# Julia-Tempering/Pigeons.jl

Hardware: AMD Instinct MI355X
Metric: replica-steps/sec (explore+swap), toy_mvn d=1024, n_chains=1024; round-trip rate (higher is better)
Workload: dtype f64

## Files before the change

pigeons.jl_amd/csrc/pte_slice8.hpp:

```cpp
#pragma once
#include "pte_slice7.hpp"

namespace pte {

#ifndef PTE_S8_BD
#define PTE_S8_BD 3
#endif
#ifndef PTE_S8_BS
#define PTE_S8_BS 9
#endif
constexpr int S8_BD = PTE_S8_BD;

#ifndef PTE_S8_WAVES
#define PTE_S8_WAVES 4
#endif
template <int NLU, int S8_BS, int WINDOW, int DBL_MODE>
__device__ __forceinline__ void slice8_body(EngineDev e, SliceParams sp, const int64_t cl) {
    using namespace s7;
    constexpr int WIN = WINDOW, REFILL_AT = WINDOW - PTE_S7_MARGIN;
    constexpr bool FAST = (DBL_MODE == 2);
    static_assert(CAP_ITERS >= S8_BS, "lane 0 must be able to run past the speculative budget");
#ifndef PTE_S8_BLK
#define PTE_S8_BLK 256
#endif
    constexpr int BLK = PTE_S8_BLK, CPB = BLK / 64;
    __shared__ struct {
        double u[WIN];
        double e[WIN];
        double x[BLK];
        double we[256];
        unsigned long long ke[256];
    } sm;
    double (&s_u)[WIN] = sm.u; double (&s_e)[WIN] = sm.e; double (&s_x)[BLK] = sm.x; double (&s_we)[256] = sm.we; unsigned long long (&s_ke)[256] = sm.ke;
    const int lane = lane_id();
#ifdef PTE_PROFILE_WAVES
    const uint64_t wave_t0 = __builtin_amdgcn_s_memrealtime();
#endif
    for (int i = lane; i < 256; i += 64) { s_we[i] = ZIG_WE[i]; s_ke[i] = ZIG_KE[i]; }
    __syncthreads();
    if (cl >= e.K) return;
    const int64_t c = e.c0 + cl;
    const int slot = e.slot_of_chain[cl];
    if (is_ref_chain(e, c)) {
        iid_refresh_recorded<NLU>(e, cl, c, slot, e.sd[c], lane);
        return;
    }
    const double lp_before = lp_before_explore(e, c, slot);
    const int64_t d = e.d;
    double *xrow = e.x + (int64_t)slot * e.ld;
    const int B = (int)((d + 63) >> 6);
    const double nhp = e.nhp[c];
    const double inv_nhp = 1.0 / nhp;
    const double inv_abs_nhp = -inv_nhp * (1.0 + 1e-6);
    const double w = sp.w;
    const double w11 = 1.1 * sp.w;
    const int cap_iters = min(sp.max_iter, CAP_ITERS);
    const int kcap = min(sp.p, 20);
    const bool shr_more = S8_BS < cap_iters;
    constexpr bool HAND_SHRINK = (S8_BS == PTE_S8_BS && S8_BS >= 6 && S8_BS <= 10);
    constexpr bool N_IS_KN = (DBL_MODE == 2) && HAND_SHRINK;

    const int hg = s7_level(lane);
    const int hrel = s7_pick(LO, hg, 0) + lane - s7_pick(BASE, hg, 0);

    const int succ_lo = s7_pick(LO, hg + 1, 0), succ_wd = s7_pick(WD, hg + 1, 0), succ_base = s7_pick(BASE, hg + 1, 0);
    const int succ_off = hrel - succ_lo;
    const int word_c = 0x10000 - succ_off;
    const int word_c9 = (1 << 20) - succ_off * 512;
    const uint64_t seed_in = e.rng[2 * slot];

    double BS = 0.0;
    for (int b = 0; b < B; ++b) {
        int64_t i = 64 * (int64_t)b + lane;
        double v = (i < d) ? xrow[i] : 0.0;
        double s = wave_sum_dpp(v * v);
        if (lane == b) BS = s;
    }
    double S = upper_tree_root<NLU>(BS);
    if (nhp * S == -INFINITY) { if (lane == 0) set_error(e, ERR_SLICE_SUPPORT, (int)c, -1); return; }

    uint64_t wseed = e.rng[2 * slot];
    const uint64_t gamma = e.rng[2 * slot + 1];
    int p = 0;
    uint64_t gamma_inv = gamma;
    for (int k = 0; k < 5; ++k) gamma_inv *= 2ull - gamma * gamma_inv;
    double wsum = 0.0;
    typedef unsigned mask2_t __attribute__((ext_vector_type(2)));
    typedef unsigned slow_mask_t __attribute__((ext_vector_type(WIN / 32)));
    slow_mask_t slow_w;
    auto fill_window = [&]() __attribute__((always_inline)) {
        __syncthreads();
        double acc = 0.0;
#pragma unroll
        for (int k = 0; k < WIN / 64; ++k) {
            const int i = 64 * k + lane;
            const uint64_t r = mix64(wseed + (uint64_t)(i + 1) * gamma);
            const uint64_t ri = r & MASK52;
            const int idx = (int)(ri & 0xFF);
            const bool fast = ri < s_ke[idx];
            const double ev = (double)ri * s_we[idx];
            s_u[i] = u52_to_unit(r);
            s_e[i] = fast ? ev : __longlong_as_double(0x7ff8000000000000LL);
            acc += fast ? ev : 0.0;
            const uint64_t sb = ballot64(!fast);
            slow_w[2 * k] = (unsigned)sb; slow_w[2 * k + 1] = (unsigned)(sb >> 32);
        }
        wsum = wave_sum_dpp(acc);
        p = 0;
        __syncthreads();
    };
    fill_window();

    int dbl_z0 = 0, dbl_z1 = 0, dbl_one_hi = 0x3ff00000;
    if constexpr (DBL_MODE == 2) asm volatile("" : "+v"(dbl_z0), "+v"(dbl_z1), "+v"(dbl_one_hi));

    long long steps_sum = 0, fb_draws = 0, ex_total = 0;
    int steps_n = 0, acc_sum = 0, acc_n = 0, n_fb = 0;
    int err = 0, err_coord = -1;
#ifdef PTE_PROFILE_SECTIONS
    long long prof[16] = {0, 0, 0, 0, 0, 0, 0, 0, 0, 0, 0, 0, 0, 0, 0, 0};
#endif

    for (int pass = 0; pass < sp.n_passes && !err; ++pass) {
        for (int b = 0; BLK * (int64_t)b < d && !err; ++b) {
            const int64_t base = BLK * (int64_t)b;
            const int nl = (int)min((int64_t)BLK, d - base);
#pragma unroll
            for (int k = 0; k < CPB; ++k) s_x[64 * k + lane] = (64 * k + lane < nl) ? xrow[base + 64 * k + lane] : 0.0;
            __builtin_amdgcn_wave_barrier();
            double Sest = S * (1.0 + 1e-6) + wsum * inv_abs_nhp;
            int l = 0, l_end = nl;
            do {
                PROF_T(t0);
                if (__builtin_expect(p > REFILL_AT, 0)) { wseed += (uint64_t)p * gamma; fill_window(); Sest = Sest * (1.0 + 1e-6) + wsum * inv_abs_nhp; }
                const bool active = (l + hg) < nl;
                const double xold = s_x[(l + hg) & (BLK - 1)];
                int idx0 = p + hrel;
                double E = s_e[idx0];
                double u0 = s_u[idx0 + 1];
                double Vd[S8_BD];
#pragma unroll
                for (int it = 0; it < S8_BD; ++it) Vd[it] = s_u[idx0 + 2 + it];
                int ex0 = 0;
                int cnt_base = 2;
                asm volatile("" : "+v"(cnt_base));
                unsigned slow_b;
                if constexpr (WIN == 512)
                    asm("s_lshr_b32 m0, %[p], 5\n" "s_nop 0\n" "s_movrels_b32 %[o], s84\n" "s_lshr_b32 %[o], %[o], %[p]"
                        : [o] "=&s"(slow_b) : [p] "s"(p), "{s[84:99]}"(slow_w) : "m0", "scc");
                else
                    asm("s_lshr_b32 m0, %[p], 5\n" "s_nop 0\n" "s_movrels_b32 %[o], s84\n" "s_lshr_b32 %[o], %[o], %[p]"
                        : [o] "=&s"(slow_b) : [p] "s"(p), "{s[84:91]}"(slow_w) : "m0", "scc");
                static_assert(WIN == 512 || WIN == 256, "the slow-path mask is sixteen or eight dwords");
                if (__builtin_expect((slow_b & 1u) != 0u, 0)) {
                    SeqRng rs{wseed + (uint64_t)p * gamma, gamma};
                    const double Ex = randexp_seq(rs);
                    const int used = (int)((rs.seed - (wseed + (uint64_t)p * gamma)) * gamma_inv);
                    if (used <= 17) {
                        ex0 = used - 1;
                        if (lane == 0) { E = Ex; idx0 += ex0; cnt_base = 2 + ex0; }
                        Sest += Ex * inv_abs_nhp;
                        ex_total += ex0;
                        u0 = s_u[idx0 + 1];
#pragma unroll
                        for (int it = 0; it < S8_BD; ++it) Vd[it] = s_u[idx0 + 2 + it];
                    }
                }
                const double Enh = E * inv_nhp;
                const double Q = __builtin_fma(xold, xold, -Enh);
                const double Bq = Sest + fabs(Q);
                double dmin = fabs(Enh);
                auto test = [&](double v) __attribute__((always_inline)) -> double {
                    const double d = __builtin_fma(v, v, -Q);
                    dmin = fmin(dmin, fabs(d));
                    return d;
                };
                double LL = xold - w * u0;
                double RR = LL + w;
                double dL = test(LL), dR = test(RR);
                int kd = 0;
                double dmin_lr = 0.0;
                unsigned need_l0 = 0u;
                uint64_t need_m = 0ull;
#if PTE_S8_BD >= 1 && PTE_S8_BD <= 4 && !defined(PTE_S8_DOUBLING_SELECTS)
                if constexpr (DBL_MODE == 2) {
                    double t_, wd_;
                    int sLh_, sRh_;
                    uint64_t sv_, sx_;
                    mask2_t sd_;
#define PTE_S8_CSTEP(V) \
                    "v_cmp_ge_f64 vcc, 0.5, " V "\n" \
                    "v_min_f64 v[102:103], v[114:115], v[116:117]\n" \
                    "v_cmpx_gt_f64_e64 %[sx], 0, v[102:103]\n" \
                    "v_add_f64 v[112:113], v[98:99], -v[96:97]\n" \
                    "v_add_u32 %[kd], 1, %[kd]\n" \
                    "v_cndmask_b32 v119, 0, %[one], vcc\n" \
                    "v_cndmask_b32 v121, %[one], v118, vcc\n" \
                    "v_fma_f64 v[96:97], -v[118:119], v[112:113], v[96:97]\n" \
                    "v_fma_f64 v[98:99], v[120:121], v[112:113], v[98:99]\n" \
                    "v_fma_f64 v[114:115], v[96:97], v[96:97], -v[110:111]\n" \
                    "v_fma_f64 v[116:117], v[98:99], v[98:99], -v[110:111]\n" \
                    "v_min_f64 v[104:105], v[104:105], |v[114:115]|\n" \
                    "v_min_f64 v[104:105], v[104:105], |v[116:117]|\n"
                    asm volatile("s_mov_b64 %[sv], exec\n"
                                 PTE_S8_CSTEP("%[V0]")
#if PTE_S8_BD >= 2
                                 PTE_S8_CSTEP("%[V1]")
#endif
#if PTE_S8_BD >= 3
                                 PTE_S8_CSTEP("%[V2]")
#endif
#if PTE_S8_BD >= 4
                                 PTE_S8_CSTEP("%[V3]")
#endif
                                 "s_mov_b64 exec, %[sv]\n"
                                 "v_min_f64 v[102:103], v[114:115], v[116:117]\n"
                                 "v_cmp_gt_f64_e64 %[sd], 0, v[102:103]\n"
                                 : "+{v[96:97]}"(LL), "+{v[98:99]}"(RR), "+{v[114:115]}"(dL), "+{v[116:117]}"(dR), "+{v[104:105]}"(dmin), [kd] "+v"(kd),
                                   "=&{v[102:103]}"(t_), "=&{v[112:113]}"(wd_), "=&{v119}"(sLh_), "=&{v121}"(sRh_), [sv] "=&s"(sv_), [sx] "=&s"(sx_), [sd] "=&s"(sd_)
                                 : "{v[110:111]}"(Q), "{v118}"(dbl_z0), "{v120}"(dbl_z1), [one] "v"(dbl_one_hi),
                                   [V0] "v"(Vd[0]), [V1] "v"(Vd[S8_BD > 1 ? 1 : 0]), [V2] "v"(Vd[S8_BD > 2 ? 2 : 0]), [V3] "v"(Vd[S8_BD > 3 ? 3 : 0])
                                 : "vcc", "scc");
#undef PTE_S8_CSTEP
                    dmin_lr = t_;
                    need_m = (uint64_t)sd_.x | ((uint64_t)sd_.y << 32); need_l0 = __builtin_amdgcn_readfirstlane(sd_.x);
                } else
                if (DBL_MODE == 1 && sp.p >= S8_BD) {
                    double t_, wd_;
                    uint64_t sv_, sv2_;
#define PTE_S8_DSTEP(V) \
                    "v_min_f64 %[t], %[dL], %[dR]\n" \
                    "v_cmp_gt_f64 vcc, 0, %[t]\n" \
                    "s_and_saveexec_b64 %[sv], vcc\n" \
                    "v_add_u32 %[kd], 1, %[kd]\n" \
                    "v_add_f64 %[wd], %[RR], -%[LL]\n" \
                    "v_cmp_ge_f64 vcc, 0.5, " V "\n" \
                    "s_and_saveexec_b64 %[sv2], vcc\n" \
                    "v_add_f64 %[LL], %[LL], -%[wd]\n" \
                    "v_fma_f64 %[dL], %[LL], %[LL], -%[Q]\n" \
                    "v_min_f64 %[dmin], %[dmin], |%[dL]|\n" \
                    "s_andn2_b64 exec, %[sv2], exec\n" \
                    "v_add_f64 %[RR], %[RR], %[wd]\n" \
                    "v_fma_f64 %[dR], %[RR], %[RR], -%[Q]\n" \
                    "v_min_f64 %[dmin], %[dmin], |%[dR]|\n" \
                    "s_mov_b64 exec, %[sv]\n"
                    asm volatile(PTE_S8_DSTEP("%[V0]")
#if PTE_S8_BD >= 2
                                 PTE_S8_DSTEP("%[V1]")
#endif
#if PTE_S8_BD >= 3
                                 PTE_S8_DSTEP("%[V2]")
#endif
#if PTE_S8_BD >= 4
                                 PTE_S8_DSTEP("%[V3]")
#endif
                                 : [LL] "+v"(LL), [RR] "+v"(RR), [dL] "+v"(dL), [dR] "+v"(dR), [dmin] "+v"(dmin), [kd] "+v"(kd),
                                   [t] "=&v"(t_), [wd] "=&v"(wd_), [sv] "=&s"(sv_), [sv2] "=&s"(sv2_)
                                 : [Q] "v"(Q), [V0] "v"(Vd[0]), [V1] "v"(Vd[S8_BD > 1 ? 1 : 0]), [V2] "v"(Vd[S8_BD > 2 ? 2 : 0]), [V3] "v"(Vd[S8_BD > 3 ? 3 : 0])
                                 : "vcc", "scc");
#undef PTE_S8_DSTEP
                } else
#endif
#pragma unroll
                for (int it = 0; it < S8_BD; ++it) {
                    const bool need = (fmin(dL, dR) < 0.0) && it < sp.p;
                    const double V = Vd[it];
                    kd += need ? 1 : 0;
                    const bool left = V <= 0.5;
                    const double wd = RR - LL;
                    if constexpr (DBL_MODE == 0) {
                        const double sL = (need && left) ? 1.0 : 0.0, sR = (need && !left) ? 1.0 : 0.0;
                        LL = __builtin_fma(-sL, wd, LL);
                        RR = __builtin_fma(sR, wd, RR);
                        dL = __builtin_fma(LL, LL, -Q);
                        dR = __builtin_fma(RR, RR, -Q);
                        dmin = fmin(dmin, fmin(fabs(dL), fabs(dR)));
                    } else {
                        const double cand = left ? (LL - wd) : (RR + wd);
                        const double dc = __builtin_fma(cand, cand, -Q);
                        dmin = need ? fmin(dmin, fabs(dc)) : dmin;
                        const bool nl_ = need && left, nr_ = need && !left;
                        LL = nl_ ? cand : LL;
                        RR = nr_ ? cand : RR;
                        dL = nl_ ? dc : dL;
                        dR = nr_ ? dc : dR;
                    }
                }
#if !(PTE_S8_BD >= 1 && PTE_S8_BD <= 4) || defined(PTE_S8_DOUBLING_SELECTS)
                static_assert(DBL_MODE != 2, "PTE_S8_DBL_MODE == 2 needs the v_cmpx doubling block: 1 <= PTE_S8_BD <= 4 and no PTE_S8_DOUBLING_SELECTS");
#endif
                if constexpr (DBL_MODE != 2) dmin_lr = fmin(dL, dR);
                unsigned more_dbl;
                if constexpr (FAST) more_dbl = need_l0 & 1u;
                else more_dbl = ballot64(lane == 0 && (dmin_lr < 0.0) && kd < kcap) != 0ull ? 1u : 0u;
                if (__builtin_expect(more_dbl != 0u, 0)) {
                    bool need = (lane == 0);
                    while (need) {
                        const double V = s_u[idx0 + 2 + kd];
                        kd += 1;
                        const bool left = V <= 0.5;
                        const double wd = RR - LL;
                        const double cand = left ? (LL - wd) : (RR + wd);
                        const double dc = test(cand);
                        LL = left ? cand : LL;
                        RR = left ? RR : cand;
                        dL = left ? dc : dL;
                        dR = left ? dR : dc;
                        need = (kd < kcap) && (fmin(dL, dR) < 0.0);
                    }
                    asm volatile("" : "+v"(dL), "+v"(dR), "+v"(kd));
                    dmin_lr = fmin(dL, dR);
                    if constexpr (FAST) {
                        dmin_lr = (kd >= sp.p) ? 0.0 : dmin_lr;
                        need_m = ballot64(dmin_lr < 0.0);
                        need_l0 = (unsigned)need_m;
                    }
                }
                const bool dbl_ok = FAST ? !__builtin_amdgcn_inverse_ballot_w64(need_m) : !((kd < sp.p) && (dmin_lr < 0.0));
                double thr2 = 1e-6 * fmax(fabs(LL), fabs(RR));
                if constexpr (DBL_MODE == 2) asm volatile("" : "+v"(thr2));
#ifdef PTE_PROFILE_SECTIONS
                asm volatile("" :: "v"(LL), "v"(RR), "v"(kd), "v"(thr2));
#endif
                PROF_T(t1); PROF_ADD(0, t1 - t0);
                const double *us = &s_u[idx0 + 2 + kd];
                double u[S8_BS];
#pragma unroll
                for (int k = 0; k < S8_BS; ++k) u[k] = us[k];
                double mthr = 2e-12 * Bq;
                int kn0 = cnt_base + kd + succ_off;
                uint64_t pre_ok;
                if constexpr (FAST) pre_ok = ballot64(active) & ~need_m;
                else pre_ok = ballot64(active && dbl_ok);
                double Lbar = LL, Rbar = RR, xf = xold, W = 0.0;
                int n = N_IS_KN ? kn0 : 0;
                if constexpr (FAST) {
                    if constexpr (N_IS_KN) asm volatile("" : "+v"(mthr), "+v"(n), "+s"(pre_ok));
                    else asm volatile("" : "+v"(mthr), "+v"(kn0), "+s"(pre_ok));
                }
                bool fin = false;
                unsigned unf_l0 = 0u;
                uint64_t unf_m = 0ull;
                if constexpr (S8_BS == PTE_S8_BS && S8_BS >= 6 && S8_BS <= 10) {
                    double t_;
                    mask2_t unf_mask;
                    uint64_t exec_save;
#define PTE_S8_STEP(U) \
                    "v_add_f64 v[112:113], v[98:99], -v[96:97]\n" \
                    "v_mul_f64 v[102:103], " U ", v[112:113]\n" \
                    "v_add_f64 v[100:101], v[96:97], v[102:103]\n" \
                    "v_cmp_lt_f64 vcc, v[100:101], v[108:109]\n" \
                    "v_fma_f64 v[102:103], v[100:101], v[100:101], -v[110:111]\n" \
                    "v_add_u32 v106, 1, v106\n" \
                    "v_cndmask_b32 v96, v96, v100, vcc\n" \
                    "v_cndmask_b32 v97, v97, v101, vcc\n" \
                    "v_cndmask_b32 v98, v100, v98, vcc\n" \
                    "v_cndmask_b32 v99, v101, v99, vcc\n" \
                    "v_min_f64 v[104:105], v[104:105], |v[102:103]|\n" \
                    "v_cmpx_ngt_f64 vcc, 0, v[102:103]\n"
                    asm volatile(".p2align 3\n"
                                 "s_mov_b64 %[sv], exec\n"
                                 PTE_S8_STEP("%[u0]") PTE_S8_STEP("%[u1]") PTE_S8_STEP("%[u2]") PTE_S8_STEP("%[u3]")
                                 PTE_S8_STEP("%[u4]") PTE_S8_STEP("%[u5]")
#if PTE_S8_BS >= 7
                                 PTE_S8_STEP("%[u6]")
#endif
#if PTE_S8_BS >= 8
                                 PTE_S8_STEP("%[u7]")
#endif
#if PTE_S8_BS >= 9
                                 PTE_S8_STEP("%[u8]")
#endif
#if PTE_S8_BS >= 10
                                 PTE_S8_STEP("%[u9]")
#endif
                                 "s_mov_b64 %[unf], exec\n"
                                 "s_mov_b64 exec, %[sv]\n"
                                 "s_nop 3\n"
                                 : "+{v[96:97]}"(Lbar), "+{v[98:99]}"(Rbar), "=&{v[100:101]}"(xf), "=&{v[102:103]}"(t_),
                                   "+{v[104:105]}"(dmin), "+{v106}"(n), "=&{v[112:113]}"(W), [unf] "=&s"(unf_mask), [sv] "=&s"(exec_save)
                                 : "{v[108:109]}"(xold), "{v[110:111]}"(Q), [u0] "v"(u[0]), [u1] "v"(u[1]), [u2] "v"(u[2]), [u3] "v"(u[3]),
                                   [u4] "v"(u[4]), [u5] "v"(u[5]), [u6] "v"(u[S8_BS > 6 ? 6 : 0]), [u7] "v"(u[S8_BS > 7 ? 7 : 0]),
                                   [u8] "v"(u[S8_BS > 8 ? 8 : 0]), [u9] "v"(u[S8_BS > 9 ? 9 : 0])
                                 : "vcc");
#undef PTE_S8_STEP
                    unf_m = (uint64_t)unf_mask.x | ((uint64_t)unf_mask.y << 32); unf_l0 = __builtin_amdgcn_readfirstlane(unf_mask.x);
                    fin = !__builtin_amdgcn_inverse_ballot_w64(unf_m);
                } else {
#pragma unroll
                    for (int k = 0; k < S8_BS; ++k) {
                        W = Rbar - Lbar;
                        const double v = Lbar + u[k] * W;
                        const double dv = __builtin_fma(v, v, -Q);
                        dmin = fmin(dmin, fabs(dv));
                        xf = fin ? xf : v;
                        n += fin ? 0 : 1;
                        const bool below = v < xold;
                        Lbar = below ? v : Lbar;
                        Rbar = below ? Rbar : v;
                        fin = fin || (dv < 0.0);
                    }
                    unf_m = ballot64(!fin);
                    unf_l0 = (unsigned)unf_m;
                }
                if (__builtin_expect((unf_l0 & 1u) != 0u, 0)) {
                  if (shr_more) {
                    double dx = 1.0;
                    bool go = (lane == 0);
                    const int n_off = N_IS_KN ? cnt_base + kd + succ_off : 0;
                    while (go) {
                        W = Rbar - Lbar;
                        xf = Lbar + us[n - n_off] * W;
                        n += 1;
                        dx = test(xf);
                        const bool below = xf < xold;
                        Lbar = below ? xf : Lbar;
                        Rbar = below ? Rbar : xf;
                        go = !(dx < 0.0) && n - n_off < cap_iters;
                    }
                    asm volatile("" : "+v"(dx), "+v"(n), "+v"(W));
                    fin = fin || (lane == 0 && dx < 0.0);
                    unf_m = ballot64(!fin);
                  }
                }
                PROF_T(t2); PROF_ADD(1, t2 - t1); PROF_ADD(3, 1);
                int gdone;
#ifdef PTE_PROFILE_SECTIONS
                constexpr bool ASM_TAIL = false;
#else
                constexpr bool ASM_TAIL = FAST && G == 5;
#endif
                if constexpr (ASM_TAIL) {
                    const int kn = N_IS_KN ? n : kn0 + n;
                    const int wsucc = ((unsigned)kn < (unsigned)succ_wd) ? kn + succ_base : 0;
                    const int word_v = (kn << 9) + word_c9 + wsucc;
                    unsigned acc; uint64_t tmask, sA_, sB_; int w_, pk_, s0_, s1_, s2_, s3_, s4_;
                    asm volatile("v_cmp_gt_f64 vcc, %[W], %[thr]\n"
                                 "v_cndmask_b32_e64 %[w], 0, %[wv], %[pre]\n"
                                 "v_cmp_gt_f64_e64 %[sA], %[dm], %[mthr]\n"
                                 "v_cndmask_b32_e64 %[w], %[w], 0, %[unf]\n"
                                 "v_cndmask_b32_e32 %[w], 0, %[w], vcc\n"
                                 "s_nop 0\n"
                                 "v_cndmask_b32_e64 %[w], 0, %[w], %[sA]\n"
                                 "v_cndmask_b32_e64 %[pk], 0, %[w], %[nz]\n"
                                 : [w] "=&v"(w_), [pk] "=&v"(pk_), [sA] "=&s"(sA_)
                                 : [wv] "v"(word_v), [pre] "s"(pre_ok), [unf] "s"(unf_m), [nz] "s"(0xFFFFFFFFFFFFFFFEull),
                                   [W] "v"(W), [thr] "v"(thr2), [dm] "v"(dmin), [mthr] "v"(mthr)
                                 : "vcc");
                    asm volatile("v_cmp_ne_u32_e64 %[sB], 0, %[w]\n"
                                 "s_mov_b64 %[tm], 1\n"
                                 "v_readlane_b32 %[s0], %[w], 0\n"
                                 "s_nop 3\n"
                                 "v_readlane_b32 %[s1], %[pk], %[s0]\n"
                                 "s_bitset1_b64 %[tm], %[s0]\n"
                                 "s_mov_b32 %[acc], %[s0]\n"
                                 "s_nop 1\n"
                                 "v_readlane_b32 %[s2], %[pk], %[s1]\n"
                                 "s_bitset1_b64 %[tm], %[s1]\n"
                                 "s_add_u32 %[acc], %[acc], %[s1]\n"
                                 "s_nop 1\n"
                                 "v_readlane_b32 %[s3], %[pk], %[s2]\n"
                                 "s_bitset1_b64 %[tm], %[s2]\n"
                                 "s_add_u32 %[acc], %[acc], %[s2]\n"
                                 "s_nop 1\n"
                                 "v_readlane_b32 %[s4], %[pk], %[s3]\n"
                                 "s_bitset1_b64 %[tm], %[s3]\n"
                                 "s_add_u32 %[acc], %[acc], %[s3]\n"
                                 "s_and_b64 %[tm], %[tm], %[sB]\n"
                                 "s_add_u32 %[acc], %[acc], %[s4]\n"
                                 : [sB] "=&s"(sB_), [tm] "=&s"(tmask), [acc] "=&s"(acc),
                                   [s0] "=&s"(s0_), [s1] "=&s"(s1_), [s2] "=&s"(s2_), [s3] "=&s"(s3_), [s4] "=&s"(s4_)
                                 : [w] "v"(w_), [pk] "v"(pk_)
                                 : "scc");
                    if (__builtin_amdgcn_inverse_ballot_w64(tmask)) s_x[(l + hg) & (BLK - 1)] = xf;
                    __builtin_amdgcn_wave_barrier();
                    p += (int)((acc >> 9) & 0x1FFu);
                    gdone = (int)((acc >> 20) & 7u);
                    l += gdone;
                } else {
                bool valid = __builtin_amdgcn_inverse_ballot_w64(pre_ok) && fin && (W > thr2);
                if constexpr (!FAST) valid = valid && !(E != E) && n <= cap_iters;
#ifdef PTE_PROFILE_SECTIONS
                asm volatile("" :: "v"(xf), "v"(n), "v"(dmin));
#endif
#ifdef PTE_PROFILE_SECTIONS
                {
                    const bool mg = dmin > 2e-12 * Bq;
                    const int rc = !active ? 7 : (E != E) ? 1 : !dbl_ok ? 2 : !fin ? 3 : !valid ? 4 : !mg ? 5 : 0;
                    const int cnt_ = N_IS_KN ? n - succ_off : cnt_base + kd + n;
                    int o_ = 0, g_ = 0, why = 0;
                    for (g_ = 0; g_ < G; ++g_) {
                        if (l + g_ >= nl) { why = 7; break; }
                        const int k_ = o_ - LO[g_];
                        if ((unsigned)k_ >= (unsigned)WD[g_]) { why = 6; break; }
                        const int ln_ = BASE[g_] + k_;
                        const int r_ = __builtin_amdgcn_readlane(rc, ln_);
                        if (r_) { why = r_; break; }
                        o_ += __builtin_amdgcn_readlane(cnt_, ln_);
                    }
                    PROF_ADD(8 + why, 1);
                }
#endif
                valid = valid && (dmin > mthr);
                const int kn = N_IS_KN ? n : kn0 + n;
                const bool inw = (unsigned)kn < (unsigned)succ_wd;
                const uint64_t vmask = ballot64(valid);
                int word_v = kn + word_c + (inw ? (int)((unsigned)(kn + succ_base) << 24) : 0);
                asm("" : "+v"(word_v));
                const int word = valid ? word_v : 0;
                const int packed = (lane != 0) ? word : 0;
#ifdef PTE_PROFILE_SECTIONS
                asm volatile("" :: "v"(packed));
#endif
                {
                    int pk = __builtin_amdgcn_readlane(word, 0);
                    unsigned acc = 0u;
                    uint64_t tmask = 1ull;
#pragma unroll
                    for (int g = 1; g < G; ++g) {
                        const int cur = (int)((unsigned)pk >> 24);
                        asm volatile("s_bitset1_b64 %0, %2\n\ts_add_u32 %1, %1, %3" : "+s"(tmask), "+s"(acc) : "s"(cur), "s"(pk) : "scc");
                        pk = __builtin_amdgcn_readlane(packed, cur);
                    }
                    acc += (unsigned)pk;
                    tmask &= vmask;
                    if (__builtin_amdgcn_inverse_ballot_w64(tmask)) s_x[(l + hg) & (BLK - 1)] = xf;
                    __builtin_amdgcn_wave_barrier();
                    p += (int)(acc & 0xFFFFu);
                    gdone = (int)((acc >> 16) & 0xFFu);
                    l += gdone;
                }
                }
#ifdef PTE_PROFILE_SECTIONS
                asm volatile("" :: "s"(p), "s"(l));
#endif
                PROF_T(t4); PROF_ADD(5, t4 - t2); PROF_ADD(4, gdone);
                if (__builtin_expect(gdone == 0, 0)) {
                    ex_total -= ex0;
                    SeqRng rs{wseed + (uint64_t)p * gamma, gamma};
                    const int ck = l >> 6, li = l & 63, bc = CPB * b + ck;
#pragma unroll
                    for (int k = 0; k < CPB; ++k) {
                        const double xk = s_x[64 * k + lane];
                        const double sk = wave_sum_dpp(xk * xk);
                        if (lane == CPB * b + k) BS = sk;
                    }
                    const double X = s_x[64 * ck + lane];
                    const double xo = readlane_f64(X, li);
                    const double E = randexp_seq(rs);
                    const double u0 = rs.rand();
                    const double Q = xo * xo - E * inv_nhp;
                    const double mg = 1e-12 * (Sest + fabs(Q));
                    const double Qlo = Q - mg, Qhi = Q + mg;
                    auto inside_exact = [&](double v) __attribute__((always_inline)) -> bool {
                        const double Xv = (lane == li) ? v : X;
                        const double sv = wave_sum_dpp(Xv * Xv), s0 = wave_sum_dpp(X * X);
                        const double Sv = upper_tree_root<NLU>((lane == bc) ? sv : BS);
                        const double S0 = upper_tree_root<NLU>((lane == bc) ? s0 : BS);
                        const double zz = nhp * S0 - E;
                        return zz < nhp * Sv;
                    };
                    auto inside = [&](double v) __attribute__((always_inline)) -> bool {
                        const double q = v * v;
                        const bool in = q < Qlo;
                        const bool out = q > Qhi;
                        if (__builtin_expect(!(in || out), 0)) return inside_exact(v);
                        return in;
                    };
                    double LL = xo - w * u0;
                    double RR = LL + w;
                    bool in_L = inside(LL), in_R = inside(RR);
                    int K = sp.p;
                    while (K > 0 && (in_L || in_R)) {
                        const double V = rs.rand();
                        if (V <= 0.5) { LL = LL - (RR - LL); in_L = inside(LL); }
                        else { RR = RR + (RR - LL); in_R = inside(RR); }
                        K -= 1;
                    }
                    steps_sum += (sp.p - K); steps_n += 1;
                    const bool doubled = (RR - LL) > w11;
                    double Lbar = LL, Rbar = RR;
                    double xn = xo;
                    bool fin = false;
                    for (int n = 1; n <= sp.max_iter; ++n) {
                        const double newpos = Lbar + rs.rand() * (Rbar - Lbar);
                        if (inside(newpos)) {
                            bool ok = true;
                            if (doubled) {
                                double Lhat = LL, Rhat = RR;
                                bool oL = !in_L, oR = !in_R;
                                bool Rstale = false, Lstale = false, D = false;
                                while (Rhat - Lhat > w11) {
                                    const double Mid = (Lhat + Rhat) / 2.0;
                                    if ((xo < Mid && newpos >= Mid) || (xo >= Mid && newpos < Mid)) D = true;
                                    if (newpos < Mid) { Rhat = Mid; Rstale = true; }
                                    else { Lhat = Mid; Lstale = true; }
                                    if (D) {
                                        if (Lstale) { oL = !inside(Lhat); Lstale = false; }
                                        if (Rstale) { oR = !inside(Rhat); Rstale = false; }
                                        if (oL && oR) { ok = false; break; }
                                    }
                                }
                            }
                            acc_n += 1;
                            if (ok) { acc_sum += 1; xn = newpos; steps_sum += n; steps_n += 1; fin = true; break; }
                        }
                        if (newpos < xo) Lbar = newpos; else Rbar = newpos;
                        if (jl_isapprox(Lbar, Rbar)) { steps_sum += n; steps_n += 1; fin = true; break; }
                    }
                    if (!fin) { err = ERR_SLICE_MAX_ITER; err_coord = (int)(base + l); l_end = 0; continue; }
                    Sest = Sest + fabs(xn * xn - xo * xo);
                    if (lane == li) s_x[l] = xn;
                    __builtin_amdgcn_wave_barrier();
                    l += 1;
                    const int used = (int)((rs.seed - (wseed + (uint64_t)p * gamma)) * gamma_inv);
                    p += used;
                    fb_draws += used; n_fb += 1;
                    PROF_T(t5); PROF_ADD(7, t5 - t4); PROF_ADD(6, 1);
                }
            } while (l < l_end);
            if (err) break;
            {
#pragma unroll
                for (int k = 0; k < CPB; ++k) {
                    const double X = s_x[64 * k + lane];
                    if (64 * k + lane < nl) xrow[base + 64 * k + lane] = X;
                    const double s = wave_sum_dpp(X * X);
                    if (lane == CPB * b + k) BS = s;
                }
                S = upper_tree_root<NLU>(BS);
                if (__builtin_expect(!isfinite(nhp * S), 0)) { err = ERR_SLICE_INVALID_LP; err_coord = (int)base; }
            }
        }
    }
    if (err) { if (lane == 0) set_error(e, err, (int)c, err_coord); return; }
    if (lane == 0) {
        const uint64_t seed_out = wseed + (uint64_t)p * gamma;
        const long long n_spec = (long long)sp.n_passes * d - n_fb;
        const long long spec_draws = (long long)((seed_out - seed_in) * gamma_inv) - fb_draws;
        steps_sum += spec_draws - ex_total - 2 * n_spec; steps_n += (int)(2 * n_spec); acc_sum += (int)n_spec; acc_n += (int)n_spec;
        e.suff[slot] = S;
        e.rng[2 * slot] = seed_out;
        e.expl_steps_sum[cl] += (double)steps_sum; e.expl_steps_n[cl] += steps_n;
        e.expl_acc_sum[cl] += (double)acc_sum;     e.expl_acc_n[cl] += acc_n;
#ifdef PTE_PROFILE_SECTIONS
        for (int i = 0; i < 16; ++i) e.on_m2[16 * cl + i] += (double)prof[i];
#endif
    }
    record_after_explore(e, cl, c, slot, lane, lp_before, S, 0.0);
#ifdef PTE_PROFILE_WAVES
    if (lane == 0) {
        double *o = e.on_m2 + 2 * (e.d + 1) + 4 * cl;
        o[0] = (double)wave_t0; o[1] = (double)__builtin_amdgcn_s_memrealtime();
        o[2] = (double)__builtin_amdgcn_s_getreg((31 << 11) | 4); o[3] = (double)__builtin_amdgcn_s_getreg((31 << 11) | 20);
    }
#endif
}

#ifndef PTE_S8_DBL_MODE
#define PTE_S8_DBL_MODE 2
#endif
template <int NLU, int S8_BS>
__global__ __launch_bounds__(64) __attribute__((amdgpu_waves_per_eu(PTE_S8_WAVES, PTE_S8_WAVES))) void k_explore_slice8(EngineDev e, SliceParams sp) {
    slice8_body<NLU, S8_BS, PTE_S7_WIN, PTE_S8_DBL_MODE>(e, sp, blockIdx.x);
}
template <int NLU, int S8_BS>
__global__ __launch_bounds__(64) __attribute__((amdgpu_waves_per_eu(PTE_S8_WAVES, PTE_S8_WAVES))) void k_explore_slice8_generic(EngineDev e, SliceParams sp) {
    slice8_body<NLU, S8_BS, PTE_S7_WIN, 0>(e, sp, blockIdx.x);
}
#ifndef PTE_S8_TWIN_WAVES
#define PTE_S8_TWIN_WAVES PTE_S8_WAVES
#endif
#ifndef PTE_S8_TWIN_FROM
#define PTE_S8_TWIN_FROM (256 * 8)
#endif
template <int NLU, int S8_BS>
__global__ __launch_bounds__(64) __attribute__((amdgpu_waves_per_eu(PTE_S8_TWIN_WAVES, PTE_S8_TWIN_WAVES))) void k_explore_slice8_lds10k(EngineDev e, SliceParams sp) {
    slice8_body<NLU, S8_BS, 256, 1>(e, sp, blockIdx.x);
}

template <int NLU, int S8_BS, int WINDOW, int DBL_MODE>
__device__ __forceinline__ void slice8_scan_loop(EngineDev e, const SliceParams &sp, const ScanLoop &sl) {
    const int lane = lane_id();
    const int64_t cl = scan_loop_chain(e.K);
    int go = 1;
    if (lane == 0) go = scan_loop_gate(sl) ? 1 : 0;
    if (!__builtin_amdgcn_readfirstlane(go)) return;
    for (int64_t i = 0; i < sl.n_scans; ++i) {
        e.trace_idx = sl.scan_idx0 + i;
        slice8_body<NLU, S8_BS, WINDOW, DBL_MODE>(e, sp, cl);
        __syncthreads();
        int slot = 0;
        if (lane == 0) slot = swap_handshake(e, sl, i, cl, e.slot_of_chain[cl]);
        slot = __builtin_amdgcn_readfirstlane(slot);
        __syncthreads();
        if (slot < 0) return;
    }
}
template <int NLU, int S8_BS>
__global__ __launch_bounds__(64) __attribute__((amdgpu_waves_per_eu(PTE_S8_WAVES, PTE_S8_WAVES))) void k_scans_slice8(EngineDev e, SliceParams sp, ScanLoop sl) {
    slice8_scan_loop<NLU, S8_BS, PTE_S7_WIN, PTE_S8_DBL_MODE>(e, sp, sl);
}
template <int NLU, int S8_BS>
__global__ __launch_bounds__(64) __attribute__((amdgpu_waves_per_eu(PTE_S8_WAVES, PTE_S8_WAVES))) void k_scans_slice8_generic(EngineDev e, SliceParams sp, ScanLoop sl) {
    slice8_scan_loop<NLU, S8_BS, PTE_S7_WIN, 0>(e, sp, sl);
}
}
```

Before: 1.598 million.

## Issue shrinkage draw LDS reads inside doubling asm and overlap with staged waits

In the fast doubling mode, the shrinkage uniforms are now read from LDS with ds_read2_b64 inside the doubling inline-asm block. The address is tracked per lane as the doubling advances. The shrinkage asm then consumes these draws behind staged lgkmcnt waits, so LDS latency overlaps with arithmetic instead of stalling before the loop. Threshold, count and active-mask setup are also folded into the asm. This adds fixed register pinning (v124-v143) and hand-scheduled waits, which raises register pressure and makes the code fragile to configuration changes.

Result: faster. 1.668 million (median of 6 runs) (+4.4%).

```diff
diff --git a/pigeons.jl_amd/csrc/pte_slice8.hpp b/pigeons.jl_amd/csrc/pte_slice8.hpp
--- a/pigeons.jl_amd/csrc/pte_slice8.hpp
+++ b/pigeons.jl_amd/csrc/pte_slice8.hpp
@@ -87,6 +87,8 @@
     double wsum = 0.0;
     typedef unsigned mask2_t __attribute__((ext_vector_type(2)));
     typedef unsigned slow_mask_t __attribute__((ext_vector_type(WIN / 32)));
+    typedef double draws8_t __attribute__((ext_vector_type(8)));
+    typedef double draws2_t __attribute__((ext_vector_type(2)));
     slow_mask_t slow_w;
     auto fill_window = [&]() __attribute__((always_inline)) {
         __syncthreads();
@@ -141,9 +143,12 @@
                 double Vd[S8_BD];
 #pragma unroll
                 for (int it = 0; it < S8_BD; ++it) Vd[it] = s_u[idx0 + 2 + it];
+                int ua = 0;
+                if constexpr (DBL_MODE == 2) ua = (int)(uintptr_t)(const __attribute__((address_space(3))) double *)&s_u[idx0];
                 int ex0 = 0;
                 int cnt_base = 2;
                 asm volatile("" : "+v"(cnt_base));
+                if constexpr (DBL_MODE == 2) asm volatile("" : "+s"(ex0));
                 unsigned slow_b;
                 if constexpr (WIN == 512)
                     asm("s_lshr_b32 m0, %[p], 5\n" "s_nop 0\n" "s_movrels_b32 %[o], s84\n" "s_lshr_b32 %[o], %[o], %[p]"
@@ -158,7 +163,7 @@
                     const int used = (int)((rs.seed - (wseed + (uint64_t)p * gamma)) * gamma_inv);
                     if (used <= 17) {
                         ex0 = used - 1;
-                        if (lane == 0) { E = Ex; idx0 += ex0; cnt_base = 2 + ex0; }
+                        if (lane == 0) { E = Ex; idx0 += ex0; cnt_base = 2 + ex0; ua += 8 * ex0; }
                         Sest += Ex * inv_abs_nhp;
                         ex_total += ex0;
                         u0 = s_u[idx0 + 1];
@@ -182,6 +187,10 @@
                 double dmin_lr = 0.0;
                 unsigned need_l0 = 0u;
                 uint64_t need_m = 0ull;
+                double thr2 = 0.0, mthr = 0.0, W = 0.0;
+                int n = 0;
+                uint64_t act_m = 0ull;
+                draws8_t ud8 = 0.0; draws2_t ud2 = 0.0;
 #if PTE_S8_BD >= 1 && PTE_S8_BD <= 4 && !defined(PTE_S8_DOUBLING_SELECTS)
                 if constexpr (DBL_MODE == 2) {
                     double t_, wd_;
@@ -194,35 +203,64 @@
                     "v_cmpx_gt_f64_e64 %[sx], 0, v[102:103]\n" \
                     "v_add_f64 v[112:113], v[98:99], -v[96:97]\n" \
                     "v_add_u32 %[kd], 1, %[kd]\n" \
+                    "v_add_u32 %[ua], 8, %[ua]\n" \
                     "v_cndmask_b32 v119, 0, %[one], vcc\n" \
                     "v_cndmask_b32 v121, %[one], v118, vcc\n" \
                     "v_fma_f64 v[96:97], -v[118:119], v[112:113], v[96:97]\n" \
                     "v_fma_f64 v[98:99], v[120:121], v[112:113], v[98:99]\n" \
                     "v_fma_f64 v[114:115], v[96:97], v[96:97], -v[110:111]\n" \
-                    "v_fma_f64 v[116:117], v[98:99], v[98:99], -v[110:111]\n" \
+                    "v_fma_f64 v[116:117], v[98:99], v[98:99], -v[110:111]\n"
+#define PTE_S8_CFOLD \
                     "v_min_f64 v[104:105], v[104:105], |v[114:115]|\n" \
                     "v_min_f64 v[104:105], v[104:105], |v[116:117]|\n"
+#if PTE_S8_BS == 6
+#define PTE_S8_UREADS_TAIL
+#elif PTE_S8_BS == 7
+#define PTE_S8_UREADS_TAIL "ds_read_b64 v[136:137], %[ua] offset:64\n"
+#elif PTE_S8_BS == 8
+#define PTE_S8_UREADS_TAIL "ds_read2_b64 v[136:139], %[ua] offset0:8 offset1:9\n"
+#elif PTE_S8_BS == 9
+#define PTE_S8_UREADS_TAIL "ds_read2_b64 v[136:139], %[ua] offset0:8 offset1:9\n" "ds_read_b64 v[140:141], %[ua] offset:80\n"
+#else
+#define PTE_S8_UREADS_TAIL "ds_read2_b64 v[136:139], %[ua] offset0:8 offset1:9\n" "ds_read2_b64 v[140:143], %[ua] offset0:10 offset1:11\n"
+#endif
                     asm volatile("s_mov_b64 %[sv], exec\n"
-                                 PTE_S8_CSTEP("%[V0]")
 #if PTE_S8_BD >= 2
-                                 PTE_S8_CSTEP("%[V1]")
+                                 PTE_S8_CSTEP("%[V0]") PTE_S8_CFOLD
 #endif
 #if PTE_S8_BD >= 3
-                                 PTE_S8_CSTEP("%[V2]")
+                                 PTE_S8_CSTEP("%[V1]") PTE_S8_CFOLD
 #endif
 #if PTE_S8_BD >= 4
-                                 PTE_S8_CSTEP("%[V3]")
-#endif
+                                 PTE_S8_CSTEP("%[V2]") PTE_S8_CFOLD
+#endif
+                                 PTE_S8_CSTEP("%[VL]")
                                  "s_mov_b64 exec, %[sv]\n"
+                                 "ds_read2_b64 v[124:127], %[ua] offset0:2 offset1:3\n"
+                                 "ds_read2_b64 v[128:131], %[ua] offset0:4 offset1:5\n"
+                                 "ds_read2_b64 v[132:135], %[ua] offset0:6 offset1:7\n"
+                                 PTE_S8_UREADS_TAIL
                                  "v_min_f64 v[102:103], v[114:115], v[116:117]\n"
                                  "v_cmp_gt_f64_e64 %[sd], 0, v[102:103]\n"
-                                 : "+{v[96:97]}"(LL), "+{v[98:99]}"(RR), "+{v[114:115]}"(dL), "+{v[116:117]}"(dR), "+{v[104:105]}"(dmin), [kd] "+v"(kd),
-                                   "=&{v[102:103]}"(t_), "=&{v[112:113]}"(wd_), "=&{v119}"(sLh_), "=&{v121}"(sRh_), [sv] "=&s"(sv_), [sx] "=&s"(sx_), [sd] "=&s"(sd_)
+                                 PTE_S8_CFOLD
+                                 "v_add_f64 %[mthr], %[Sest], |v[110:111]|\n"
+                                 "v_max_f64 %[thr], |v[96:97]|, |v[98:99]|\n"
+                                 "v_cmp_gt_i32_e64 %[act], %[nl], %[lg]\n"
+                                 "v_add3_u32 v106, %[cb], %[so], %[kd]\n"
+                                 "v_mul_f64 %[mthr], %[mthr], %[c_m]\n"
+                                 "v_mul_f64 %[thr], %[thr], %[c_t]\n"
+                                 "v_add_f64 v[112:113], v[98:99], -v[96:97]\n"
+                                 : "+{v[96:97]}"(LL), "+{v[98:99]}"(RR), "+{v[114:115]}"(dL), "+{v[116:117]}"(dR), "+{v[104:105]}"(dmin), [kd] "+v"(kd), [ua] "+v"(ua),
+                                   "=&{v[102:103]}"(t_), "=&{v[112:113]}"(wd_), "=&{v119}"(sLh_), "=&{v121}"(sRh_), [sv] "=&s"(sv_), [sx] "=&s"(sx_), [sd] "=&s"(sd_),
+                                   "=&{v[124:139]}"(ud8), "=&{v[140:143]}"(ud2), [mthr] "=&v"(mthr), [thr] "=&v"(thr2), "=&{v106}"(n), [act] "=&s"(act_m)
                                  : "{v[110:111]}"(Q), "{v118}"(dbl_z0), "{v120}"(dbl_z1), [one] "v"(dbl_one_hi),
-                                   [V0] "v"(Vd[0]), [V1] "v"(Vd[S8_BD > 1 ? 1 : 0]), [V2] "v"(Vd[S8_BD > 2 ? 2 : 0]), [V3] "v"(Vd[S8_BD > 3 ? 3 : 0])
+                                   [V0] "v"(Vd[0]), [V1] "v"(Vd[S8_BD > 2 ? 1 : 0]), [V2] "v"(Vd[S8_BD > 3 ? 2 : 0]), [VL] "v"(Vd[S8_BD - 1]),
+                                   [Sest] "v"(Sest), [nl] "s"(nl), [lg] "v"(l + hg), [cb] "v"(cnt_base), [so] "v"(succ_off), [c_m] "s"(2e-12), [c_t] "s"(1e-6)
                                  : "vcc", "scc");
 #undef PTE_S8_CSTEP
-                    dmin_lr = t_;
+#undef PTE_S8_CFOLD
+#undef PTE_S8_UREADS_TAIL
+                    dmin_lr = t_; W = wd_;
                     need_m = (uint64_t)sd_.x | ((uint64_t)sd_.y << 32); need_l0 = __builtin_amdgcn_readfirstlane(sd_.x);
                 } else
                 if (DBL_MODE == 1 && sp.p >= S8_BD) {
@@ -314,30 +352,37 @@
                         dmin_lr = (kd >= sp.p) ? 0.0 : dmin_lr;
                         need_m = ballot64(dmin_lr < 0.0);
                         need_l0 = (unsigned)need_m;
+                        thr2 = 1e-6 * fmax(fabs(LL), fabs(RR));
+                        n = cnt_base + kd + succ_off;
+                        W = RR - LL;
+                        const double *un = &s_u[idx0 + 2 + kd];
+#pragma unroll
+                        for (int k = 0; k < 8; ++k) ud8[k] = (k < S8_BS) ? un[k] : 0.0;
+#pragma unroll
+                        for (int k = 8; k < 10; ++k) ud2[k - 8] = (k < S8_BS) ? un[k] : 0.0;
+                        asm volatile("" : "+{v[124:139]}"(ud8), "+{v[140:143]}"(ud2));
                     }
                 }
                 const bool dbl_ok = FAST ? !__builtin_amdgcn_inverse_ballot_w64(need_m) : !((kd < sp.p) && (dmin_lr < 0.0));
-                double thr2 = 1e-6 * fmax(fabs(LL), fabs(RR));
-                if constexpr (DBL_MODE == 2) asm volatile("" : "+v"(thr2));
+                if constexpr (DBL_MODE != 2) thr2 = 1e-6 * fmax(fabs(LL), fabs(RR));
 #ifdef PTE_PROFILE_SECTIONS
                 asm volatile("" :: "v"(LL), "v"(RR), "v"(kd), "v"(thr2));
 #endif
                 PROF_T(t1); PROF_ADD(0, t1 - t0);
+                static_assert(DBL_MODE != 2 || HAND_SHRINK, "PTE_S8_DBL_MODE == 2 hands its draws to the hand-written shrinkage block: 6 <= PTE_S8_BS <= 10");
                 const double *us = &s_u[idx0 + 2 + kd];
                 double u[S8_BS];
-#pragma unroll
-                for (int k = 0; k < S8_BS; ++k) u[k] = us[k];
-                double mthr = 2e-12 * Bq;
+                if constexpr (DBL_MODE != 2) {
+#pragma unroll
+                    for (int k = 0; k < S8_BS; ++k) u[k] = us[k];
+                }
+                if constexpr (DBL_MODE != 2) mthr = 2e-12 * Bq;
                 int kn0 = cnt_base + kd + succ_off;
                 uint64_t pre_ok;
-                if constexpr (FAST) pre_ok = ballot64(active) & ~need_m;
+                if constexpr (FAST) pre_ok = 0ull;
                 else pre_ok = ballot64(active && dbl_ok);
-                double Lbar = LL, Rbar = RR, xf = xold, W = 0.0;
-                int n = N_IS_KN ? kn0 : 0;
-                if constexpr (FAST) {
-                    if constexpr (N_IS_KN) asm volatile("" : "+v"(mthr), "+v"(n), "+s"(pre_ok));
-                    else asm volatile("" : "+v"(mthr), "+v"(kn0), "+s"(pre_ok));
-                }
+                double Lbar = LL, Rbar = RR, xf = xold;
+                if constexpr (!N_IS_KN) n = 0;
                 bool fin = false;
                 unsigned unf_l0 = 0u;
                 uint64_t unf_m = 0ull;
@@ -345,8 +390,10 @@
                     double t_;
                     mask2_t unf_mask;
                     uint64_t exec_save;
-#define PTE_S8_STEP(U) \
-                    "v_add_f64 v[112:113], v[98:99], -v[96:97]\n" \
+#define PTE_S8_STEP_W \
+                    "v_add_f64 v[112:113], v[98:99], -v[96:97]\n"
+#define PTE_S8_STEP(U) PTE_S8_STEP_W PTE_S8_STEP_U(U)
+#define PTE_S8_STEP_U(U) \
                     "v_mul_f64 v[102:103], " U ", v[112:113]\n" \
                     "v_add_f64 v[100:101], v[96:97], v[102:103]\n" \
                     "v_cmp_lt_f64 vcc, v[100:101], v[108:109]\n" \
@@ -358,6 +405,60 @@
                     "v_cndmask_b32 v99, v101, v99, vcc\n" \
                     "v_min_f64 v[104:105], v[104:105], |v[102:103]|\n" \
                     "v_cmpx_ngt_f64 vcc, 0, v[102:103]\n"
+                    if constexpr (DBL_MODE == 2) {
+#if defined(PTE_S8_ONE_WAIT) || defined(PTE_PROFILE_SECTIONS)
+#define PTE_S8_WAIT(K) "s_waitcnt lgkmcnt(0)\n"
+#else
+#define PTE_S8_WAIT(K) "s_waitcnt lgkmcnt(" #K ")\n"
+#endif
+#if PTE_S8_BS >= 9
+#define PTE_S8_W1 4
+#define PTE_S8_W3 3
+#define PTE_S8_W5 2
+#define PTE_S8_W7 1
+#elif PTE_S8_BS >= 7
+#define PTE_S8_W1 3
+#define PTE_S8_W3 2
+#define PTE_S8_W5 1
+#define PTE_S8_W7 0
+#else
+#define PTE_S8_W1 2
+#define PTE_S8_W3 1
+#define PTE_S8_W5 0
+#endif
+#define PTE_S8_WAIT_(K) PTE_S8_WAIT(K)
+                    asm volatile(".p2align 3\n"
+                                 "s_mov_b64 %[sv], exec\n"
+                                 "s_andn2_b64 %[pre], %[act], %[need]\n"
+                                 PTE_S8_WAIT_(PTE_S8_W1) PTE_S8_STEP_U("v[124:125]") PTE_S8_STEP("v[126:127]")
+                                 PTE_S8_STEP_W PTE_S8_WAIT_(PTE_S8_W3) PTE_S8_STEP_U("v[128:129]") PTE_S8_STEP("v[130:131]")
+                                 PTE_S8_STEP_W PTE_S8_WAIT_(PTE_S8_W5) PTE_S8_STEP_U("v[132:133]") PTE_S8_STEP("v[134:135]")
+#if PTE_S8_BS >= 7
+                                 PTE_S8_STEP_W PTE_S8_WAIT_(PTE_S8_W7) PTE_S8_STEP_U("v[136:137]")
+#endif
+#if PTE_S8_BS >= 8
+                                 PTE_S8_STEP("v[138:139]")
+#endif
+#if PTE_S8_BS >= 9
+                                 PTE_S8_STEP_W PTE_S8_WAIT_(0) PTE_S8_STEP_U("v[140:141]")
+#endif
+#if PTE_S8_BS >= 10
+                                 PTE_S8_STEP("v[142:143]")
+#endif
+                                 "s_mov_b64 %[unf], exec\n"
+                                 "s_mov_b64 exec, %[sv]\n"
+                                 "s_nop 3\n"
+                                 : "+{v[96:97]}"(Lbar), "+{v[98:99]}"(Rbar), "=&{v[100:101]}"(xf), "=&{v[102:103]}"(t_),
+                                   "+{v[104:105]}"(dmin), "+{v106}"(n), "+{v[112:113]}"(W), [unf] "=&s"(unf_mask), [sv] "=&s"(exec_save), [pre] "=&s"(pre_ok)
+                                 : "{v[108:109]}"(xold), "{v[110:111]}"(Q), "{v[124:139]}"(ud8), "{v[140:143]}"(ud2), [act] "s"(act_m), [need] "s"(need_m)
+                                 : "vcc", "scc");
+#undef PTE_S8_WAIT
+#undef PTE_S8_WAIT_
+#undef PTE_S8_W1
+#undef PTE_S8_W3
+#undef PTE_S8_W5
+#undef PTE_S8_W7
+                    } else
                     asm volatile(".p2align 3\n"
                                  "s_mov_b64 %[sv], exec\n"
                                  PTE_S8_STEP("%[u0]") PTE_S8_STEP("%[u1]") PTE_S8_STEP("%[u2]") PTE_S8_STEP("%[u3]")
@@ -384,6 +485,8 @@
                                    [u8] "v"(u[S8_BS > 8 ? 8 : 0]), [u9] "v"(u[S8_BS > 9 ? 9 : 0])
                                  : "vcc");
 #undef PTE_S8_STEP
+#undef PTE_S8_STEP_W
+#undef PTE_S8_STEP_U
                     unf_m = (uint64_t)unf_mask.x | ((uint64_t)unf_mask.y << 32); unf_l0 = __builtin_amdgcn_readfirstlane(unf_mask.x);
                     fin = !__builtin_amdgcn_inverse_ballot_w64(unf_m);
                 } else {
```
